# martende/findex

Measured on NVIDIA B200. Metric: fm_count_queries_per_s_len16_1GB_text, higher is better.
Workload: dtype u32

## Files before the change

findex_b200/csrc/fmx_device.cuh:

```cuda
#pragma once
#include <cstdint>
#include <cuda_runtime.h>

#include "../../include/fmgpu.h"

namespace fmx {

constexpr uint32_t kBitsPerBlock = 480;
constexpr int kCodeAbsent = 0xFF;

struct DevIndex {
    const uint4   *blocks;
    uint64_t       stride;
    const uint8_t *bwt;
    const uint32_t *C;
    const uint32_t *base;
    const uint8_t *code;
    const uint4   *mark;
    const uint32_t *samples;
    const uint4   *bm;
    uint32_t n, eof;
    int32_t  layout, levels;
    uint32_t z[8];
    int32_t  wmx_b, wmx_levels;
// ... 384 lines not shown
__device__ __forceinline__ bool dict_chain(const DevIndex &ix, const uint8_t *code, PatFn pat, int &i, uint32_t &sp, uint32_t &ep,
                                           uint32_t &touched, uint32_t &steps, int depth, bool top_known_missed = false) {
    const int Jc = ix.dict_Jc;
    const uint32_t bits = (uint32_t)ix.dict_bits;
    for (int t = (depth - ix.dict_D) / Jc + 1; t <= kDictMaxTiers && i >= 0 && depth < ix.dict_Dx; ++t) {
        const int j = (i + 1) < Jc ? (i + 1) : Jc;
        uint64_t syms = 0;
        bool ok = true;
        for (int k = 0; k < j; ++k) {
            const uint32_t c = pat(i - k), cd = code[c];
            ok = ok && (cd != (uint32_t)kCodeAbsent) && (c != 0);
            syms |= (uint64_t)cd << (bits * (uint32_t)k);
        }
        if (!ok) return true;
        uint32_t s, e;
        if (!top_known_missed && dict_probe<G, STATS>(ix, dict_chain_key(sp, j, t, syms), s, e, touched)) {
            sp = s; ep = e;
            i -= j;
            depth += j;
            if (STATS) steps += j;
            if (j < Jc) return true;
            continue;
        }
        if (!BISECT) return false;
        int lo = 0, hi = j - 1;
        uint32_t bs = 0, be = 0;
        const uint32_t psp = sp;
        while (lo < hi) {
            const int mid = (lo + hi + 1) >> 1;
            if (dict_probe<G, STATS>(ix, dict_chain_key(psp, mid, t, syms & ((1ull << (bits * (uint32_t)mid)) - 1ull)), s, e, touched)) { lo = mid; bs = s; be = e; }
            else hi = mid - 1;
        }
        if (lo > 0) { sp = bs; ep = be; i -= lo; if (STATS) steps += lo; }
        return true;
    }
    return true;
}

struct CtxQuery {
    unsigned long long qlo, qhi, mlo, mhi;
    uint32_t sh;
    bool zero, absent;
};
template <typename PatFn>
__device__ __forceinline__ CtxQuery ctx_query(const DevIndex &ix, const SharedTables &tb, PatFn pat, int j, int o) {
    CtxQuery q;
    const uint32_t bits = (uint32_t)ix.isat_bits;
    q.qlo = 0; q.qhi = 0;
    q.sh = (uint32_t)(ix.ctx_J - j) * bits;
    const uint32_t nb = (uint32_t)j * bits;
    q.mlo = nb >= 64 ? ~0ull : ((1ull << nb) - 1ull);
    q.mhi = nb <= 64 ? 0ull : ((1ull << (nb - 64)) - 1ull);
    q.zero = false; q.absent = false;
    if (ix.ctx_raw) {
        uint32_t w0, w1, w2;
        pat.bytes12(o, w0, w1, w2);
        q.qlo = ((unsigned long long)w1 << 32) | w0;
        q.qhi = w2;
        const unsigned long long l = q.qlo | ~q.mlo, h = (q.qhi & q.mhi) | ~q.mhi;
        q.zero = (((l - 0x0101010101010101ull) & ~l) | ((h - 0x0101010101010101ull) & ~h)) & 0x8080808080808080ull;
    } else {
        for (int k = 0; k < j; ++k) {
            const uint32_t pc = pat(o + k), cd = tb.code[pc];
            q.zero = q.zero || (pc == 0);
            q.absent = q.absent || (cd == (uint32_t)kCodeAbsent);
            const unsigned long long v = (unsigned long long)((cd + 1u) & ((1u << bits) - 1u));
            const uint32_t ob = (uint32_t)k * bits;
            if (ob < 64) { q.qlo |= v << ob; if (ob + bits > 64) q.qhi |= v >> (64 - ob); }
            else q.qhi |= v << (ob - 64);
        }
    }
    return q;
}
__device__ __forceinline__ bool ctx_match(const CtxQuery &q, const uint4 &b) {
    const unsigned long long elo = ((unsigned long long)b.z << 32) | b.y, ehi = b.w;
    unsigned long long lo, hi;
    if (q.sh == 0) { lo = elo; hi = ehi; }
    else if (q.sh < 64) { lo = (elo >> q.sh) | (ehi << (64 - q.sh)); hi = ehi >> q.sh; }
    else { lo = ehi >> (q.sh - 64); hi = 0; }
    return (((lo ^ q.qlo) & q.mlo) | ((hi ^ q.qhi) & q.mhi)) == 0ull;
}

constexpr uint32_t kKmerGroup = 8, kKmerWide = 0xFFu, kKmerInlineRows = 3;

template <int G, bool STATS, typename PatFn>
__device__ __forceinline__ void kmer_group(const DevIndex &ix, const SharedTables &tb, PatFn pat, bool fetch, uint32_t idx, int &i,
                                           uint32_t &sp, uint32_t &ep, uint32_t &touched, uint32_t &steps, uint32_t &pre_from,
                                           uint32_t &pre_best, uint32_t &pre_cnt) {
    const uint4 *blk = reinterpret_cast<const uint4 *>(ix.kmer) + (uint64_t)(idx / kKmerGroup) * 4;
    uint4 q0, q1, q2, q3;
    if constexpr (G == 1) {
        const uint32_t odd = threadIdx.x & 1u;
        const unsigned long long mine = reinterpret_cast<unsigned long long>(blk);
        const unsigned long long pe = __shfl_sync(0xFFFFFFFFu, mine, (threadIdx.x & 31u) & ~1u);
        const unsigned long long po = __shfl_sync(0xFFFFFFFFu, mine, (threadIdx.x & 31u) | 1u);
        const bool fe = __shfl_sync(0xFFFFFFFFu, fetch, (threadIdx.x & 31u) & ~1u), fo = __shfl_sync(0xFFFFFFFFu, fetch, (threadIdx.x & 31u) | 1u);
        uint4 x0 = make_uint4(0, 0, 0, 0), x1 = x0, y0 = x0, y1 = x0;
        if (fe) ldg256(reinterpret_cast<const uint4 *>(pe) + 2 * odd, x0, x1);
        if (fo) ldg256(reinterpret_cast<const uint4 *>(po) + 2 * odd, y0, y1);
        uint4 s0 = odd ? x0 : y0, s1 = odd ? x1 : y1;
        s0.x = __shfl_xor_sync(0xFFFFFFFFu, s0.x, 1); s0.y = __shfl_xor_sync(0xFFFFFFFFu, s0.y, 1);
        s0.z = __shfl_xor_sync(0xFFFFFFFFu, s0.z, 1); s0.w = __shfl_xor_sync(0xFFFFFFFFu, s0.w, 1);
        s1.x = __shfl_xor_sync(0xFFFFFFFFu, s1.x, 1); s1.y = __shfl_xor_sync(0xFFFFFFFFu, s1.y, 1);
        s1.z = __shfl_xor_sync(0xFFFFFFFFu, s1.z, 1); s1.w = __shfl_xor_sync(0xFFFFFFFFu, s1.w, 1);
        if (odd) { q0 = s0; q1 = s1; q2 = y0; q3 = y1; } else { q0 = x0; q1 = x1; q2 = s0; q3 = s1; }
    } else {
        if (!fetch) return;
        ldg256(blk, q0, q1);
        ldg256(blk + 2, q2, q3);
    }
    if (!fetch) return;
    const uint32_t e = idx % kKmerGroup, kind = q0.w >> 24, base = q0.x;
    uint32_t lo, hi;
    if (kind != kKmerWide) {
        const unsigned long long ends = ((unsigned long long)q0.z << 32) | q0.y;
        hi = base + (uint32_t)((ends >> (8 * e)) & 0xFFu);
        lo = base + (e ? (uint32_t)((ends >> (8 * e - 8)) & 0xFFu) : 0u);
    } else {
        auto end_of = [&](uint32_t k) {
            return k < 4 ? (k < 2 ? (k == 0 ? q1.x : q1.y) : (k == 2 ? q1.z : q1.w)) : (k < 6 ? (k == 4 ? q2.x : q2.y) : (k == 6 ? q2.z : q2.w));
        };
        hi = end_of(e);
        lo = (e ? end_of(e - 1) : base) + (((e < 4 ? q3.x : q3.y) >> (8 * (e & 3))) & 0xFFu);
    }
    if (lo < hi) { sp = lo; ep = hi; } else { sp = 0; ep = 0; }
    if (STATS) { touched += 1; steps += ix.kmer_k; }
    if (kind == kKmerWide || kind == 0 || ix.ctx == nullptr || sp >= ep || i < 0) return;
    const int rem = i + 1;
    const uint32_t rows = ep - sp;
    const int t = rem <= kCtxPlanMax ? (int)tb.plan[rem] : kCtxHops - 1;
    const uint32_t need = rem <= kCtxPlanMax ? (uint32_t)tb.plan[128 + rem] : (uint32_t)(rem / ix.ctx_J + 3);
    if (t != kCtxHops - 1 || rows > kCtxMaxRows || !(rows == 1u || rows * need <= (uint32_t)rem)) return;
    const int j = ix.ctx_J;
    const CtxQuery q = ctx_query(ix, tb, pat, j, rem - j);
    if (q.zero) return;
    uint32_t best = 0xFFFFFFFFu, cnt = 0;
#pragma unroll
    for (uint32_t k = 0; k < kKmerInlineRows; ++k) {
        const uint4 &pl = k == 0 ? q1 : k == 1 ? q2 : q3;
        if (k < kind && base + k >= sp && base + k < ep && !q.absent && ctx_match(q, pl)) { best = pl.x < best ? pl.x : best; ++cnt; }
    }
    if (ep <= base + kind) {
        if (cnt) { sp = best; ep = best + cnt; } else { sp = 0; ep = 0; }
        i -= j;
        if (STATS) steps += j;
    } else {
        const int lane = (G == 1) ? 0 : (threadIdx.x & (G - 1));
        pre_from = base + kind;
        pre_best = best;
        pre_cnt = lane == 0 ? cnt : 0u;
    }
}

constexpr int kSearchFresh = 0, kSearchTopMissed = 1, kSearchResume = 2, kSearchChainMissed = 3;
template <int G, int LAYOUT, bool STATS, typename PatFn>
__device__ __forceinline__ void search_pattern(const DevIndex &ix, const SharedTables &tb, PatFn pat, int len, bool active,
                                               uint32_t &sp, uint32_t &ep, uint32_t &touched, uint32_t &steps,
                                               int mode = kSearchFresh, uint32_t rsp = 0, uint32_t rep = 0, int rconsumed = 0) {
    const int lane = (G == 1) ? 0 : (threadIdx.x & (G - 1));
    const uint32_t gmask = group_mask<G>();
    sp = 0;
    ep = active ? ix.n : 0u;
    int i = len - 1;
    bool noshort = (ix.isat == nullptr);
    uint32_t pre_from = 0, pre_best = 0xFFFFFFFFu, pre_cnt = 0;
    bool kfetch = false;
    uint32_t kidx = 0;
    if (active && (mode == kSearchResume || mode == kSearchChainMissed)) {
        sp = rsp; ep = rep;
        i -= rconsumed;
        if (mode == kSearchChainMissed) dict_chain<G, STATS, true>(ix, tb.code, pat, i, sp, ep, touched, steps, rconsumed, true);
    } else if (active && i >= 0) {
        bool done = false;
        if (ix.dict != nullptr && len > ix.kmer_k) {
            const int K = ix.kmer_k;
            const uint32_t bits = (uint32_t)ix.dict_bits;
            int hi = len < ix.dict_D ? len : ix.dict_D;
            uint64_t full = 0;
            bool ok = true;
            for (int j = 0; j < hi; ++j) {
                const uint32_t c = pat(len - 1 - j), code = tb.code[c];
                ok = ok && (code != (uint32_t)kCodeAbsent) && (c != 0);
                full |= (uint64_t)code << (bits * (uint32_t)j);
            }
            if (ok) {
                int lo = K, d = hi;
                uint32_t bsp = 0, bep = 0;
                if (mode == kSearchTopMissed) { --hi; d = (lo + hi + 1) >> 1; }
                while (lo < hi) {
                    uint32_t s, e;
                    if (dict_probe<G, STATS>(ix, dict_key(full, d, bits), s, e, touched)) { lo = d; bsp = s; bep = e; }
                    else hi = d - 1;
                    d = (lo + hi + 1) >> 1;
                }
                if (lo > K) {
                    sp = bsp; ep = bep;
                    i -= lo;
                    done = true;
                    if (STATS) steps += lo;
                    if (lo == ix.dict_D && ix.dict_Dx > ix.dict_D) dict_chain<G, STATS, true>(ix, tb.code, pat, i, sp, ep, touched, steps, lo);
                }
            }
        }
        if (!done && ix.kmer != nullptr && len >= ix.kmer_k) {
            const int K = ix.kmer_k;
            uint32_t idx = 0;
            bool ok = true;
            for (int j = 0; j < K; ++j) {
                const uint32_t c = pat(ix.kmer_rows ? len - K + j : len - 1 - j), code = tb.code[c];
                ok = ok && (code != (uint32_t)kCodeAbsent) && (c != 0);
                idx = idx * ix.kmer_sigma + code;
            }
            if (ok) {
                i -= K;
                done = true;
                if (ix.kmer_rows) { kfetch = true; kidx = idx; }
                else {
                    const uint2 v = ldg64(ix.kmer + idx);
                    sp = v.x; ep = v.y;
                    if (STATS) { touched += 1; steps += K; }
                }
            }
        }
        if (!done) {
            const uint32_t c = pat(i);
            sp = tb.C[c];
            ep = tb.C[c + 1];
            --i;
            if (STATS) ++steps;
        }
    }
    if (ix.kmer != nullptr && ix.kmer_rows) kmer_group<G, STATS>(ix, tb, pat, kfetch, kidx, i, sp, ep, touched, steps, pre_from, pre_best, pre_cnt);
    bool noctx = (ix.ctx == nullptr && ix.ctx8 == nullptr);
    for (;;) {
        const bool go = (i >= 0) && (sp < ep);
        if (go) {
            bool stepped = false;
            const int rem = i + 1;
            if (!noctx && ix.ctx8 != nullptr && (ep - sp) <= kCtxMaxRows && rem >= ix.ctx8_J) {
                const int J = ix.ctx8_J, o = rem - J;
                uint32_t q = 0;
                bool zero = false, absent = false;
                for (int k = 0; k < J; ++k) {
                    const uint32_t pc = pat(o + k), cd = tb.code[pc];
                    zero = zero || (pc == 0);
                    absent = absent || (cd == (uint32_t)kCodeAbsent);
                    q |= (cd & 3u) << (2 * k);
                }
                if (zero) noctx = true;
                else {
                    uint32_t best = 0xFFFFFFFFu, cnt = 0;
                    if (!absent) {
                        for (uint32_t r = sp + (uint32_t)lane; r < ep; r += G) {
                            const uint2 e = ldg64(ix.ctx8 + r);
                            if (e.y == q && e.x != 0xFFFFFFFFu) { best = e.x < best ? e.x : best; ++cnt; }
                        }
                    }
                    if (STATS && lane == 0) { touched += absent ? 0u : ep - sp; steps += J; }
                    if (G >= 2) { best = min(best, __shfl_xor_sync(gmask, best, 1)); cnt += __shfl_xor_sync(gmask, cnt, 1); }
                    if (G >= 4) { best = min(best, __shfl_xor_sync(gmask, best, 2)); cnt += __shfl_xor_sync(gmask, cnt, 2); }
                    if (cnt) { sp = best; ep = best + cnt; } else { sp = 0; ep = 0; }
                    i -= J;
                    stepped = true;
                }
            }
            if (!stepped && !noctx && ix.ctx != nullptr && (ep - sp) <= kCtxMaxRows) {
                const uint32_t rows = ep - sp;
                const int t = rem <= kCtxPlanMax ? (int)tb.plan[rem] : kCtxHops - 1;
                const uint32_t need = rem <= kCtxPlanMax ? (uint32_t)tb.plan[128 + rem] : (uint32_t)(rem / ix.ctx_J + 3);
                if (rows == 1u || rows * need <= (uint32_t)rem) {
                    const int j = (int)tb.hops[t];
                    const CtxQuery q = ctx_query(ix, tb, pat, j, rem - j);
                    if (q.zero) noctx = true;
                    else {
                        const uint32_t from = sp > pre_from ? sp : pre_from;
                        uint32_t best = pre_best, cnt = pre_cnt;
                        if (!q.absent) {
                            for (uint32_t r = from + (uint32_t)lane; r < ep; r += G) {
                                uint4 a, b;
                                ldg256(ix.ctx + (uint64_t)r * 2, a, b);
                                if (ctx_match(q, b)) {
                                    const uint32_t row = t == 0 ? a.x : t == 1 ? a.y : t == 2 ? a.z : t == 3 ? a.w : b.x;
                                    best = row < best ? row : best;
                                    ++cnt;
                                }
                            }
                        }
                        pre_from = 0; pre_best = 0xFFFFFFFFu; pre_cnt = 0;
                        if (STATS && lane == 0) { touched += q.absent ? 0u : ep - from; steps += j; }
                        if (G >= 2) { best = min(best, __shfl_xor_sync(gmask, best, 1)); cnt += __shfl_xor_sync(gmask, cnt, 1); }
                        if (G >= 4) { best = min(best, __shfl_xor_sync(gmask, best, 2)); cnt += __shfl_xor_sync(gmask, cnt, 2); }
                        if (cnt) { sp = best; ep = best + cnt; } else { sp = 0; ep = 0; }
                        i -= j;
                        stepped = true;
                    }
                }
            }
            if (!stepped && !noshort && (ep - sp) == 1u && i >= 2 && i < ix.isat_syms) {
                const uint32_t q = ldg32(ix.sa + sp);
                const bool fits = q >= (uint32_t)rem;
                const uint32_t b0 = fits ? q - (uint32_t)rem : 0u;
                const uint4 e = ldg128(ix.isat + b0);
                const uint32_t bits = (uint32_t)ix.isat_bits, fmask = (1u << bits) - 1u;
                bool eq = fits, zero = false;
                for (int k = lane; k < rem; k += G) {
                    const uint32_t pc = pat(k);
                    const uint32_t o = (uint32_t)k * bits, w = o >> 5;
                    const uint32_t lo = w == 0 ? e.y : w == 1 ? e.z : e.w, hi = w == 0 ? e.z : w == 1 ? e.w : 0u;
                    const uint32_t sym = __funnelshift_r(lo, hi, o & 31u) & fmask;
                    zero = zero || (pc == 0);
                    eq = eq && (sym == (uint32_t)tb.code[pc] + 1u);
                }
                if (G > 1) { eq = __all_sync(gmask, eq); zero = __any_sync(gmask, zero); }
                if (zero) noshort = true;
                else {
                    if (eq) { sp = e.x; ep = e.x + 1; } else { sp = 0; ep = 0; }
                    i = -1;
                    stepped = true;
                    if (STATS) { touched += 2; steps += rem; }
                }
            }
            if (!stepped) {
                backward_step<G, LAYOUT, STATS>(ix, tb, pat(i), sp, ep, touched);
                --i;
                if (STATS) ++steps;
            }
        }
        if (__all_sync(0xFFFFFFFFu, !go)) break;
    }
}

template <int G, int LAYOUT>
__device__ __forceinline__ uint32_t lf_value(const DevIndex &ix, const SharedTables &t, uint32_t c, uint32_t pos) {
    const uint32_t code = t.code[c];
    if (c == 0) return pos > ix.eof ? 1u : 0u;
    if (code == kCodeAbsent) return t.C[c];
    if (LAYOUT == FMX_LAYOUT_PLANES) {
        return t.base[c] + rank_one<G>(ix.blocks + (uint64_t)code * ix.stride * 4, pos, nullptr);
    } else if (LAYOUT == FMX_LAYOUT_WMX) {
        uint32_t p = pos;
        const int b = ix.wmx_b, L = ix.wmx_levels;
        for (int l = 0; l < L; ++l) {
            const uint32_t d = (code >> (b * (L - 1 - l))) & ((1u << b) - 1u);
            p = ix.zx[l][d] + rank_one_x<G>(ix.blocks + (uint64_t)l * ix.wmx_stride * 8, b, d, p);
        }
        if (code == 0) p -= (pos > ix.eof);
        return t.base[c] + p;
    } else {
        uint32_t p = pos;
        const int L = ix.levels;
        for (int l = 0; l < L; ++l) {
            uint32_t r = rank_one<G>(ix.blocks + (uint64_t)l * ix.stride * 4, p, nullptr);
            if ((code >> (L - 1 - l)) & 1u) p = ix.z[l] + r; else p -= r;
        }
        if (code == 0) p -= (pos > ix.eof);
        return t.base[c] + p;
    }
}

}
```

findex_b200/csrc/fmx_kernels.cu:

```cuda
#include "fmx_kernels.cuh"

#include <algorithm>

namespace fmx {

template <int G, int LAYOUT, bool STATS, typename OutT, int MINB = (LAYOUT == FMX_LAYOUT_WMX ? 5 : (G == 1) ? 6 : 8)>
__global__ void __launch_bounds__(kThreads, MINB)
count_fixed_kernel(const __grid_constant__ DevIndex ix, const uint8_t *__restrict__ pat, int len, long long m,
                   OutT *__restrict__ sp_out, OutT *__restrict__ ep_out, unsigned long long *stats, const __grid_constant__ PeerSinks sinks) {
    __shared__ SharedTables tb;
    extern __shared__ __align__(16) uint8_t spat[];
    constexpr int QPB = kThreads / G;
    load_tables(tb, ix);

    const long long q0 = (long long)blockIdx.x * QPB;
    const int nq = (int)((m - q0) < (long long)QPB ? (m - q0) : (long long)QPB);
    {
        const uint8_t *src = pat + q0 * len;
        const int nbytes = nq * len;
        if ((reinterpret_cast<uintptr_t>(src) & 15) == 0) {
            const int nvec = nbytes >> 4;
            for (int i = threadIdx.x; i < nvec; i += kThreads)
                reinterpret_cast<uint4 *>(spat)[i] = ldg128(reinterpret_cast<const uint4 *>(src) + i);
            for (int i = (nvec << 4) + threadIdx.x; i < nbytes; i += kThreads) spat[i] = src[i];
        } else {
            for (int i = threadIdx.x; i < nbytes; i += kThreads) spat[i] = src[i];
        }
    }
    __syncthreads();

    const int g = threadIdx.x / G;
    const bool active = g < nq;
    uint32_t sp, ep, touched = 0, steps = 0;
    search_pattern<G, LAYOUT, STATS>(ix, tb, SmemPattern{spat + g * len, len, (len & 3) == 0}, len, active, sp, ep, touched, steps);
    const bool hit = sp < ep;
    const uint32_t cnt = hit ? ep - sp : 0u;
    if (active && (threadIdx.x % G) == 0) {
        sp_out[q0 + g] = hit ? (OutT)sp : (OutT)0;
        ep_out[q0 + g] = hit ? (OutT)ep : (OutT)0;
        if (sinks.n == 1) sinks.p[0][sinks.offset + q0 + g] = cnt;
    }
    if (sinks.n > 1) {
        __shared__ __align__(16) uint32_t scnt[kThreads];
        if ((threadIdx.x % G) == 0) scnt[g] = active ? cnt : 0u;
        __syncthreads();
        const long long base = sinks.offset + q0;
        if (nq == QPB && (base & 3) == 0) {
            constexpr int V = QPB / 4;
            for (int w = threadIdx.x; w < sinks.n * V; w += kThreads) {
                const int j = w / V, k = w - j * V;
                reinterpret_cast<uint4 *>(sinks.p[j] + base)[k] = reinterpret_cast<const uint4 *>(scnt)[k];
            }
        } else {
            for (int w = threadIdx.x; w < sinks.n * nq; w += kThreads) {
                const int j = w / nq, k = w - j * nq;
                sinks.p[j][base + k] = scnt[k];
            }
        }
    }
    if (STATS) {
        if ((threadIdx.x % G) != 0) { touched = 0; steps = 0; }
        for (int o = 16; o; o >>= 1) {
            touched += __shfl_xor_sync(0xFFFFFFFFu, touched, o);
            steps += __shfl_xor_sync(0xFFFFFFFFu, steps, o);
        }
        if ((threadIdx.x & 31) == 0) { atomicAdd(&stats[0], (unsigned long long)touched); atomicAdd(&stats[1], (unsigned long long)steps); }
    }
}

template <int G, int LAYOUT, typename OutT>
__global__ void __launch_bounds__(kThreads)
count_fixed_gmem_kernel(const __grid_constant__ DevIndex ix, const uint8_t *__restrict__ pat, int len, long long m, OutT *__restrict__ sp_out,
                        OutT *__restrict__ ep_out, const __grid_constant__ PeerSinks sinks) {
    __shared__ SharedTables tb;
    load_tables(tb, ix);
    __syncthreads();
    constexpr int QPB = kThreads / G;
    const long long q = (long long)blockIdx.x * QPB + threadIdx.x / G;
    const bool active = q < m;
    uint32_t sp, ep, touched = 0, steps = 0;
    search_pattern<G, LAYOUT, false>(ix, tb, GlobalPattern{pat + (active ? q : 0) * len, len}, len, active, sp, ep, touched, steps);
    if (active && (threadIdx.x % G) == 0) {
        const bool hit = sp < ep;
        sp_out[q] = hit ? (OutT)sp : (OutT)0;
        ep_out[q] = hit ? (OutT)ep : (OutT)0;
        for (int j = 0; j < sinks.n; ++j) sinks.p[j][sinks.offset + q] = hit ? ep - sp : 0u;
    }
}

constexpr uint32_t kListModeShift = 30, kListIdMask = (1u << kListModeShift) - 1u;

template <typename OutT>
__global__ void __launch_bounds__(kThreads)
count_dict_first_kernel(const __grid_constant__ DevIndex ix, const uint8_t *__restrict__ pat, int len, long long m, OutT *__restrict__ sp_out,
                        OutT *__restrict__ ep_out, uint2 *__restrict__ list, unsigned long long *__restrict__ list_count,
                        const __grid_constant__ PeerSinks sinks) {
    __shared__ uint8_t scode[256];
    extern __shared__ __align__(16) uint8_t spat[];
    for (int i = threadIdx.x; i < 256; i += kThreads) scode[i] = ix.code[i];
    const int d0 = len < ix.dict_D ? len : ix.dict_D;
    const long long q0 = (long long)blockIdx.x * kThreads;
    const int nq = (int)((m - q0) < (long long)kThreads ? (m - q0) : (long long)kThreads);
    {
        const uint8_t *src = pat + q0 * len;
        const int nbytes = nq * len;
        if ((reinterpret_cast<uintptr_t>(src) & 15) == 0) {
            const int nvec = nbytes >> 4;
            for (int i = threadIdx.x; i < nvec; i += kThreads)
                reinterpret_cast<uint4 *>(spat)[i] = ldg128(reinterpret_cast<const uint4 *>(src) + i);
            for (int i = (nvec << 4) + threadIdx.x; i < nbytes; i += kThreads) spat[i] = src[i];
        } else {
            for (int i = threadIdx.x; i < nbytes; i += kThreads) spat[i] = src[i];
        }
    }
    __syncthreads();
    const bool active = (int)threadIdx.x < nq;
    const long long q = q0 + threadIdx.x;
    uint32_t entry = 0xFFFFFFFFu, consumed = 0;
    if (active) {
        const uint8_t *p = spat + (size_t)threadIdx.x * len;
        const uint32_t bits = (uint32_t)ix.dict_bits;
        uint64_t full = 0;
        bool ok = true;
        for (int j = 0; j < d0; ++j) {
            const uint32_t c = p[len - 1 - j], code = scode[c];
            ok = ok && (code != (uint32_t)kCodeAbsent) && (c != 0);
            full |= (uint64_t)code << (bits * (uint32_t)j);
        }
        entry = (uint32_t)threadIdx.x | ((uint32_t)kSearchFresh << kListModeShift);
        if (ok) {
            uint32_t s = 0, e = 0, touched = 0;
            if (dict_probe<1, false>(ix, dict_key(full, d0, bits), s, e, touched)) {
                int i = len - 1 - d0;
                bool chain_open = true;
                if (i >= 0 && ix.dict_Dx > ix.dict_D) {
                    uint32_t steps = 0;
                    chain_open = dict_chain<1, false, false>(ix, scode, SmemPattern{p, len, false}, i, s, e, touched, steps, d0);
                }
                consumed = (uint32_t)(len - 1 - i);
                sp_out[q] = (OutT)s;
                ep_out[q] = (OutT)e;
                if (i < 0) {
                    entry = 0xFFFFFFFFu;
                    for (int j = 0; j < sinks.n; ++j) sinks.p[j][sinks.offset + q] = e - s;
                } else entry = (uint32_t)threadIdx.x | ((uint32_t)(chain_open ? kSearchResume : kSearchChainMissed) << kListModeShift);
            } else entry = (uint32_t)threadIdx.x | ((uint32_t)kSearchTopMissed << kListModeShift);
        }
    }
    __shared__ uint32_t wcount[kThreads / 32];
    __shared__ unsigned long long cta_base;
    const uint32_t need = __ballot_sync(0xFFFFFFFFu, entry != 0xFFFFFFFFu);
    const int lane = threadIdx.x & 31, warp = threadIdx.x >> 5;
    if (lane == 0) wcount[warp] = (uint32_t)__popc(need);
    __syncthreads();
    if (threadIdx.x == 0) {
        uint32_t total = 0;
        for (int w = 0; w < kThreads / 32; ++w) { const uint32_t c = wcount[w]; wcount[w] = total; total += c; }
        cta_base = total ? atomicAdd(list_count, (unsigned long long)total) : 0ull;
    }
    __syncthreads();
    if (entry != 0xFFFFFFFFu) {
        const uint32_t mode = entry >> kListModeShift;
        list[cta_base + wcount[warp] + __popc(need & ((1u << lane) - 1u))] = make_uint2((uint32_t)(q0 + (entry & kListIdMask)) | (mode << kListModeShift), consumed);
    }
}

template <int G, int LAYOUT, typename OutT>
__global__ void __launch_bounds__(kThreads)
count_list_kernel(const __grid_constant__ DevIndex ix, const uint8_t *__restrict__ pat, int len, OutT *__restrict__ sp_out, OutT *__restrict__ ep_out,
                  const uint2 *__restrict__ list, const unsigned long long *__restrict__ list_count, const __grid_constant__ PeerSinks sinks) {
    __shared__ SharedTables tb;
    extern __shared__ __align__(16) uint8_t spat[];
    constexpr int QPB = kThreads / G;
    const unsigned long long count = *list_count;
    if ((unsigned long long)blockIdx.x * QPB >= count) return;
    load_tables(tb, ix);
    const int g = threadIdx.x / G, lane = threadIdx.x % G;
    const int stride = (len + 3) & ~3;
    {
        const unsigned long long t = (unsigned long long)blockIdx.x * QPB + g;
        const bool active = t < count;
        const uint2 le = active ? list[t] : make_uint2(0u, 0u);
        const uint32_t entry = le.x;
        const long long q = (long long)(entry & kListIdMask);
        const int mode = (int)(entry >> kListModeShift);
        __syncthreads();
        if (active) {
            const uint8_t *src = pat + q * len;
            uint8_t *dst = spat + (size_t)g * stride;
            if ((len & 3) == 0 && (reinterpret_cast<uintptr_t>(src) & 3) == 0)
                for (int w = lane; w < (len >> 2); w += G) reinterpret_cast<uint32_t *>(dst)[w] = __ldg(reinterpret_cast<const uint32_t *>(src) + w);
            else
                for (int b = lane; b < len; b += G) dst[b] = __ldg(src + b);
        }
        __syncthreads();
        uint32_t rsp = 0, rep = 0;
        if (active && (mode == kSearchResume || mode == kSearchChainMissed)) { rsp = (uint32_t)sp_out[q]; rep = (uint32_t)ep_out[q]; }
        uint32_t sp, ep, touched = 0, steps = 0;
        search_pattern<G, LAYOUT, false>(ix, tb, SmemPattern{spat + (size_t)g * stride, len, true}, len, active, sp, ep, touched, steps, mode, rsp, rep, (int)le.y);
        if (active && (threadIdx.x % G) == 0) {
            const bool hit = sp < ep;
            sp_out[q] = hit ? (OutT)sp : (OutT)0;
            ep_out[q] = hit ? (OutT)ep : (OutT)0;
            for (int j = 0; j < sinks.n; ++j) sinks.p[j][sinks.offset + q] = hit ? ep - sp : 0u;
        }
    }
}

template <int G, int LAYOUT>
__global__ void __launch_bounds__(kThreads)
count_var_kernel(const __grid_constant__ DevIndex ix, const uint8_t *__restrict__ pat, const long long *__restrict__ off,
                 long long m, long long *__restrict__ sp_out, long long *__restrict__ ep_out) {
    __shared__ SharedTables tb;
    load_tables(tb, ix);
    __syncthreads();
    constexpr int QPB = kThreads / G;
    const long long q = (long long)blockIdx.x * QPB + threadIdx.x / G;
    const bool active = q < m;
    long long lo = 0, hi = 0;
// ... 177 lines not shown
        if (++k > ix.n) { FMX_EMIT(0xFFFFFFFFu); return; }
    }
#undef FMX_EMIT
}

template <typename OutT>
__global__ void key_positions_kernel(const unsigned long long *__restrict__ key, long long n, OutT *__restrict__ out) {
    const long long i = (long long)blockIdx.x * blockDim.x + threadIdx.x;
    if (i < n) out[i] = (OutT)(key[i] & 0xFFFFFFFFull);
}
cudaError_t launch_key_positions(const uint64_t *d_key, int64_t n, uint32_t *d_out32, int64_t *d_out64, cudaStream_t st) {
    if (n <= 0) return cudaSuccess;
    const unsigned grid = (unsigned)((n + 255) / 256);
    if (d_out32) key_positions_kernel<uint32_t><<<grid, 256, 0, st>>>((const unsigned long long *)d_key, n, d_out32);
    else key_positions_kernel<long long><<<grid, 256, 0, st>>>((const unsigned long long *)d_key, n, (long long *)d_out64);
    return cudaGetLastError();
}

__global__ void unpack2_kernel(const uint8_t *__restrict__ codes, int len, long long m, uint32_t alpha4, uint8_t *__restrict__ out) {
    const int pb = (len + 3) >> 2;
    const long long t = (long long)blockIdx.x * blockDim.x + threadIdx.x;
    if (t >= m * pb) return;
    const long long q = t / pb;
    const int b = (int)(t - q * pb);
    const uint32_t c = codes[t];
    uint8_t *dst = out + q * len + 4 * b;
#pragma unroll
    for (int j = 0; j < 4; ++j)
        if (4 * b + j < len) dst[j] = (uint8_t)(alpha4 >> (8 * ((c >> (2 * j)) & 3u)));
}
cudaError_t launch_unpack2(const uint8_t *d_codes, int len, int64_t m, uint32_t alpha4, uint8_t *d_out, cudaStream_t st) {
    const int64_t total = m * ((len + 3) / 4);
    if (total > 0) unpack2_kernel<<<(unsigned)((total + 255) / 256), 256, 0, st>>>(d_codes, len, m, alpha4, d_out);
    return cudaGetLastError();
}

__global__ void interval_len_kernel(const uint32_t *__restrict__ sp, const uint32_t *__restrict__ ep, long long m, long long *__restrict__ out) {
    const long long q = (long long)blockIdx.x * blockDim.x + threadIdx.x;
    if (q > m) return;
    out[q] = (q < m && ep[q] > sp[q]) ? (long long)(ep[q] - sp[q]) : 0ll;
}
cudaError_t launch_interval_len(const uint32_t *d_sp, const uint32_t *d_ep, int64_t m, int64_t *d_out, cudaStream_t st) {
    interval_len_kernel<<<(unsigned)((m + 1 + 255) / 256), 256, 0, st>>>(d_sp, d_ep, m, (long long *)d_out);
    return cudaGetLastError();
}

__global__ void __launch_bounds__(256)
scatter_words_kernel(const uint32_t *__restrict__ src, long long count, const __grid_constant__ PeerSinks sinks, const long long *__restrict__ d_dst_off,
                     long long dst_scale) {
    const long long dst0 = sinks.offset + (d_dst_off ? *d_dst_off * dst_scale : 0ll);
    const long long stride = (long long)gridDim.x * blockDim.x, tid = (long long)blockIdx.x * blockDim.x + threadIdx.x;
    if (((reinterpret_cast<uintptr_t>(src) | (uintptr_t)(dst0 * 4)) & 15) == 0) {
        const long long nv = count >> 2;
        for (long long i = tid; i < nv; i += stride) {
            const uint4 v = reinterpret_cast<const uint4 *>(src)[i];
            for (int j = 0; j < sinks.n; ++j) reinterpret_cast<uint4 *>(sinks.p[j] + dst0)[i] = v;
        }
        for (long long i = (nv << 2) + tid; i < count; i += stride) { const uint32_t v = src[i]; for (int j = 0; j < sinks.n; ++j) sinks.p[j][dst0 + i] = v; }
    } else {
        for (long long i = tid; i < count; i += stride) { const uint32_t v = src[i]; for (int j = 0; j < sinks.n; ++j) sinks.p[j][dst0 + i] = v; }
    }
}
cudaError_t launch_scatter_words(const uint32_t *d_src, int64_t count, const PeerSinks &sinks, const int64_t *d_dst_off, int64_t dst_scale, cudaStream_t st) {
    if (count <= 0 || sinks.n <= 0) return cudaSuccess;
    const unsigned grid = (unsigned)std::min<int64_t>((count / 4 + 255) / 256 + 1, 148 * 8);
    scatter_words_kernel<<<grid, 256, 0, st>>>(d_src, count, sinks, (const long long *)d_dst_off, dst_scale);
    return cudaGetLastError();
}

template <int LANES, int VEC>
__global__ void __launch_bounds__(kThreads)
gather_kernel(const uint4 *__restrict__ base, unsigned long long n_units, long long gathers, int chain, uint32_t seed,
              unsigned long long *sink) {
    const long long gid = ((long long)blockIdx.x * kThreads + threadIdx.x) / LANES;
    const int lane = threadIdx.x % LANES;
    if (gid >= gathers) return;
    unsigned long long x = (unsigned long long)gid * 0x9E3779B97F4A7C15ull + seed;
    uint32_t acc = 0;
    for (int s = 0; s < chain; ++s) {
        x ^= x >> 33; x *= 0xFF51AFD7ED558CCDull; x ^= x >> 33; x *= 0xC4CEB9FE1A85EC53ull; x ^= x >> 33;
        const unsigned long long unit = __umul64hi(x, n_units);
        const uint4 *p = base + unit * (LANES * VEC) + lane * VEC;
        uint32_t v = 0;
#pragma unroll
        for (int i = 0; i < VEC; ++i) { const uint4 q = ldg128(p + i); v ^= q.x ^ q.y ^ q.z ^ q.w; }
        if (LANES > 1) {
            const uint32_t mask = ((LANES == 32) ? 0xFFFFFFFFu : ((1u << LANES) - 1u)) << ((threadIdx.x & 31) & ~(LANES - 1));
            for (int o = 1; o < LANES; o <<= 1) v ^= __shfl_xor_sync(mask, v, o);
        }
        acc ^= v;
        x += v;
    }
    if (acc == 0x12345678u && lane == 0) atomicAdd(sink, 1ull);
}

#define FMX_DISPATCH(cfg, CALL)                                                                      \
    do {                                                                                             \
        if ((cfg).layout == FMX_LAYOUT_PLANES) {                                                     \
            if ((cfg).lanes == 1) { CALL(1, FMX_LAYOUT_PLANES); }                                    \
            else if ((cfg).lanes == 2) { CALL(2, FMX_LAYOUT_PLANES); }                               \
            else { CALL(4, FMX_LAYOUT_PLANES); }                                                     \
        } else if ((cfg).layout == FMX_LAYOUT_WMX) {                                                 \
            if ((cfg).lanes == 1) { CALL(1, FMX_LAYOUT_WMX); }                                       \
            else if ((cfg).lanes == 2) { CALL(2, FMX_LAYOUT_WMX); }                                  \
            else { CALL(4, FMX_LAYOUT_WMX); }                                                        \
        } else {                                                                                     \
            if ((cfg).lanes == 1) { CALL(1, FMX_LAYOUT_WM); }                                        \
            else if ((cfg).lanes == 2) { CALL(2, FMX_LAYOUT_WM); }                                   \
            else { CALL(4, FMX_LAYOUT_WM); }                                                         \
        }                                                                                            \
    } while (0)

static inline unsigned grid_for(int64_t items, int lanes) {
    const int64_t per = kThreads / lanes;
    return (unsigned)((items + per - 1) / per);
}

cudaError_t launch_count_fixed(const DevIndex &ix, LaunchCfg cfg, const uint8_t *d_pat, int len, int64_t m, void *d_sp,
                               void *d_ep, bool out64, unsigned long long *d_stats, cudaStream_t st, const PeerSinks *sinks_or_null) {
    if (m <= 0) return cudaSuccess;
    if (cfg.count_lanes) cfg.lanes = cfg.count_lanes;
    PeerSinks sinks{};
    if (sinks_or_null) sinks = *sinks_or_null;
    const size_t smem = (size_t)(kThreads / cfg.lanes) * (size_t)(len > 0 ? len : 1) + 16;
    const bool too_long = smem > 160 * 1024;
    if (ix.dict != nullptr && len > ix.kmer_k && len <= ix.dict_Dx && !d_stats && m < (1ll << kListModeShift) && (size_t)kThreads * (size_t)len <= 160 * 1024) {
        unsigned long long *cnt = nullptr;
        cudaError_t e = cudaMallocAsync(&cnt, 16 + (size_t)m * 8, st);
        if (e != cudaSuccess) return e;
        uint2 *list = reinterpret_cast<uint2 *>(cnt + 2);
        cudaMemsetAsync(cnt, 0, 8, st);
        const size_t smem1 = (size_t)kThreads * (size_t)len;
        const unsigned grid1 = grid_for(m, 1);
        if (out64) {
            auto k = count_dict_first_kernel<long long>;
            cudaFuncSetAttribute(k, cudaFuncAttributeMaxDynamicSharedMemorySize, (int)smem1);
            k<<<grid1, kThreads, smem1, st>>>(ix, d_pat, len, m, (long long *)d_sp, (long long *)d_ep, list, cnt, sinks);
        } else {
            auto k = count_dict_first_kernel<uint32_t>;
            cudaFuncSetAttribute(k, cudaFuncAttributeMaxDynamicSharedMemorySize, (int)smem1);
            k<<<grid1, kThreads, smem1, st>>>(ix, d_pat, len, m, (uint32_t *)d_sp, (uint32_t *)d_ep, list, cnt, sinks);
        }
        const unsigned grid2 = grid_for(m, cfg.lanes);
#define CALL2(G, LAY)                                                                                                  \
        {                                                                                                              \
            const size_t smem2 = (size_t)(kThreads / G) * (size_t)((len + 3) & ~3) + 16;                               \
            if (out64) count_list_kernel<G, LAY, long long><<<grid2, kThreads, smem2, st>>>(ix, d_pat, len, (long long *)d_sp, (long long *)d_ep, list, cnt, sinks); \
            else count_list_kernel<G, LAY, uint32_t><<<grid2, kThreads, smem2, st>>>(ix, d_pat, len, (uint32_t *)d_sp, (uint32_t *)d_ep, list, cnt, sinks); \
        }
        FMX_DISPATCH(cfg, CALL2);
#undef CALL2
        cudaFreeAsync(cnt, st);
        return cudaGetLastError();
    }
#define CALL(G, LAY)                                                                                                  \
    {                                                                                                                 \
        if (too_long && !d_stats) {                                                                                   \
            if (out64) count_fixed_gmem_kernel<G, LAY, long long><<<grid_for(m, G), kThreads, 0, st>>>(ix, d_pat, len, m, (long long *)d_sp, (long long *)d_ep, sinks); \
            else count_fixed_gmem_kernel<G, LAY, uint32_t><<<grid_for(m, G), kThreads, 0, st>>>(ix, d_pat, len, m, (uint32_t *)d_sp, (uint32_t *)d_ep, sinks); \
        } else if (too_long) {                                                                                        \
            return cudaErrorInvalidValue;                                                                             \
        } else if (d_stats) {                                                                                                \
            auto k = count_fixed_kernel<G, LAY, true, uint32_t>;                                                      \
            cudaFuncSetAttribute(k, cudaFuncAttributeMaxDynamicSharedMemorySize, (int)smem);                          \
            k<<<grid_for(m, G), kThreads, smem, st>>>(ix, d_pat, len, m, (uint32_t *)d_sp, (uint32_t *)d_ep, d_stats, sinks); \
        } else if (out64) {                                                                                           \
            auto k = count_fixed_kernel<G, LAY, false, long long>;                                                    \
            cudaFuncSetAttribute(k, cudaFuncAttributeMaxDynamicSharedMemorySize, (int)smem);                          \
            k<<<grid_for(m, G), kThreads, smem, st>>>(ix, d_pat, len, m, (long long *)d_sp, (long long *)d_ep, nullptr, sinks); \
        } else if (cfg.min_blocks >= 4 && cfg.min_blocks <= 8) {                      \
            auto k = cfg.min_blocks == 4 ? count_fixed_kernel<G, LAY, false, uint32_t, 4> : cfg.min_blocks == 5 ? count_fixed_kernel<G, LAY, false, uint32_t, 5> : \
                     cfg.min_blocks == 6 ? count_fixed_kernel<G, LAY, false, uint32_t, 6> : cfg.min_blocks == 7 ? count_fixed_kernel<G, LAY, false, uint32_t, 7> : \
                     count_fixed_kernel<G, LAY, false, uint32_t, 8>;                                                  \
            cudaFuncSetAttribute(k, cudaFuncAttributeMaxDynamicSharedMemorySize, (int)smem);                          \
            k<<<grid_for(m, G), kThreads, smem, st>>>(ix, d_pat, len, m, (uint32_t *)d_sp, (uint32_t *)d_ep, nullptr, sinks); \
        } else {                                                                                                      \
            auto k = count_fixed_kernel<G, LAY, false, uint32_t>;                                                     \
            cudaFuncSetAttribute(k, cudaFuncAttributeMaxDynamicSharedMemorySize, (int)smem);                          \
            k<<<grid_for(m, G), kThreads, smem, st>>>(ix, d_pat, len, m, (uint32_t *)d_sp, (uint32_t *)d_ep, nullptr, sinks); \
        }                                                                                                             \
    }
    FMX_DISPATCH(cfg, CALL);
#undef CALL
    return cudaGetLastError();
}

cudaError_t launch_count_var(const DevIndex &ix, LaunchCfg cfg, const uint8_t *d_pat, const int64_t *d_off, int64_t m,
                             int64_t *d_sp, int64_t *d_ep, cudaStream_t st) {
    if (m <= 0) return cudaSuccess;
    if (cfg.count_lanes) cfg.lanes = cfg.count_lanes;
#define CALL(G, LAY) count_var_kernel<G, LAY><<<grid_for(m, G), kThreads, 0, st>>>(ix, d_pat, (const long long *)d_off, m, (long long *)d_sp, (long long *)d_ep)
    FMX_DISPATCH(cfg, CALL);
#undef CALL
    return cudaGetLastError();
}

cudaError_t launch_occ(const DevIndex &ix, LaunchCfg cfg, const uint8_t *d_c, const int64_t *d_key, int64_t m, int64_t *d_out,
                       cudaStream_t st) {
    if (m <= 0) return cudaSuccess;
#define CALL(G, LAY) occ_kernel<G, LAY><<<grid_for(m, G), kThreads, 0, st>>>(ix, d_c, (const long long *)d_key, m, (long long *)d_out)
    FMX_DISPATCH(cfg, CALL);
#undef CALL
    return cudaGetLastError();
}

cudaError_t launch_prev_range(const DevIndex &ix, LaunchCfg cfg, const int64_t *d_sp, const int64_t *d_ep, const uint8_t *d_c,
                              int64_t m, int64_t *d_sp1, int64_t *d_ep1, cudaStream_t st) {
    if (m <= 0) return cudaSuccess;
#define CALL(G, LAY) prev_range_kernel<G, LAY><<<grid_for(m, G), kThreads, 0, st>>>(ix, (const long long *)d_sp, (const long long *)d_ep, d_c, m, (long long *)d_sp1, (long long *)d_ep1)
    FMX_DISPATCH(cfg, CALL);
#undef CALL
    return cudaGetLastError();
}

cudaError_t launch_interval_prev_range(const DevIndex &ix, LaunchCfg cfg, int64_t sp, int64_t ep, int cstart, int cend,
                                       int64_t *d_sp1, int64_t *d_ep1, cudaStream_t st) {
    const int64_t m = cend - cstart + 1;
    if (m <= 0) return cudaSuccess;
#define CALL(G, LAY) interval_prev_range_kernel<G, LAY><<<grid_for(m, G), kThreads, 0, st>>>(ix, (uint32_t)sp, (uint32_t)ep, cstart, cend, (long long *)d_sp1, (long long *)d_ep1)
    FMX_DISPATCH(cfg, CALL);
#undef CALL
    return cudaGetLastError();
}

cudaError_t launch_lf(const DevIndex &ix, LaunchCfg cfg, const int64_t *d_row, int64_t m, int64_t *d_out, cudaStream_t st) {
    if (m <= 0) return cudaSuccess;
#define CALL(G, LAY) lf_kernel<G, LAY><<<grid_for(m, G), kThreads, 0, st>>>(ix, (const long long *)d_row, m, (long long *)d_out)
    FMX_DISPATCH(cfg, CALL);
#undef CALL
    return cudaGetLastError();
}

cudaError_t launch_prev_substr(const DevIndex &ix, LaunchCfg cfg, const int64_t *d_row, int64_t m, int len, uint8_t *d_out,
                               cudaStream_t st) {
    if (m <= 0 || len <= 0) return cudaSuccess;
#define CALL(G, LAY) prev_substr_kernel<G, LAY><<<grid_for(m, G), kThreads, 0, st>>>(ix, (const long long *)d_row, m, len, d_out)
    FMX_DISPATCH(cfg, CALL);
#undef CALL
    return cudaGetLastError();
}

cudaError_t launch_fl(const DevIndex &ix, LaunchCfg cfg, const int64_t *d_row, int64_t m, int64_t *d_out, cudaStream_t st) {
    if (m <= 0) return cudaSuccess;
#define CALL(G, LAY) fl_kernel<G, LAY><<<grid_for(m, G), kThreads, 0, st>>>(ix, (const long long *)d_row, m, (long long *)d_out)
    FMX_DISPATCH(cfg, CALL);
#undef CALL
    return cudaGetLastError();
}

cudaError_t launch_next_substr(const DevIndex &ix, LaunchCfg cfg, const int64_t *d_row, int64_t m, int len, uint8_t *d_out,
                               int *d_out_len, cudaStream_t st) {
    if (m <= 0) return cudaSuccess;
#define CALL(G, LAY) next_substr_kernel<G, LAY><<<grid_for(m, G), kThreads, 0, st>>>(ix, (const long long *)d_row, m, len, d_out, d_out_len)
    FMX_DISPATCH(cfg, CALL);
#undef CALL
    return cudaGetLastError();
}

cudaError_t launch_locate(const DevIndex &ix, LaunchCfg cfg, const uint32_t *d_sp, const int64_t *d_off, int64_t q0, int64_t q1,
                          int64_t t0, int64_t count, uint32_t *d_pos, uint64_t *d_key, unsigned long long *d_steps, cudaStream_t st) {
    if (count <= 0) return cudaSuccess;
#define CALL(G, LAY) locate_kernel<G, LAY><<<grid_for(count, G), kThreads, 0, st>>>(ix, d_sp, (const long long *)d_off, q0, q1, t0, count, d_pos, (unsigned long long *)d_key, d_steps)
    FMX_DISPATCH(cfg, CALL);
#undef CALL
    return cudaGetLastError();
}

cudaError_t launch_gather_bench(const uint4 *base, uint64_t n_blocks64, int bytes, int lanes, int64_t gathers, int chain,
                                uint32_t seed, unsigned long long *d_sink, cudaStream_t st) {
    const int per_lane = bytes / lanes;
    if (per_lane < 16 || per_lane % 16 || (per_lane / 16) > 8 || lanes < 1 || lanes > 32 || (lanes & (lanes - 1))) return cudaErrorInvalidValue;
    const int vec = per_lane / 16;
    const unsigned long long units = n_blocks64 * 64ull / (unsigned long long)bytes;
    const unsigned grid = (unsigned)((gathers * lanes + kThreads - 1) / kThreads);
#define GK(L, V) gather_kernel<L, V><<<grid, kThreads, 0, st>>>(base, units, gathers, chain, seed, d_sink)
    if (vec == 1) { switch (lanes) { case 1: GK(1, 1); break; case 2: GK(2, 1); break; case 4: GK(4, 1); break; case 8: GK(8, 1); break; case 16: GK(16, 1); break; default: GK(32, 1); } }
    else if (vec == 2) { switch (lanes) { case 1: GK(1, 2); break; case 2: GK(2, 2); break; case 4: GK(4, 2); break; case 8: GK(8, 2); break; default: return cudaErrorInvalidValue; } }
    else if (vec == 4) { switch (lanes) { case 1: GK(1, 4); break; case 2: GK(2, 4); break; case 4: GK(4, 4); break; default: return cudaErrorInvalidValue; } }
    else if (vec == 8) { switch (lanes) { case 1: GK(1, 8); break; case 2: GK(2, 8); break; default: return cudaErrorInvalidValue; } }
    else return cudaErrorInvalidValue;
#undef GK
    return cudaGetLastError();
}

}
```

Measured before the change: 27.40 billion.

## Add persistent warp kernel that compacts unfinished queries into a queue

Adds a persistent count kernel in which each warp stages tiles of 32 patterns into shared memory with cp.async double buffering. It resolves each pattern's k-mer prefix, writes finished queries immediately, and compacts the remaining ones into a per-warp queue. The backward search runs only when 32 queued queries are ready, so all lanes stay busy. The goal is to cut warp divergence from queries that finish early and to overlap pattern loads with compute, at the cost of extra shared memory and queue bookkeeping.

Measured after the change: 28.36 billion, median of 6. 1.03x the previous value.

```diff
diff --git a/findex_b200/csrc/fmx_device.cuh b/findex_b200/csrc/fmx_device.cuh
--- a/findex_b200/csrc/fmx_device.cuh
+++ b/findex_b200/csrc/fmx_device.cuh
@@ -560,85 +560,25 @@
     }
 }
 
-constexpr int kSearchFresh = 0, kSearchTopMissed = 1, kSearchResume = 2, kSearchChainMissed = 3;
+template <typename PatFn>
+__device__ __forceinline__ bool kmer_entry(const DevIndex &ix, const SharedTables &tb, PatFn pat, int len, uint32_t &idx) {
+    const int K = ix.kmer_k;
+    idx = 0;
+    bool ok = true;
+    for (int j = 0; j < K; ++j) {
+        const uint32_t c = pat(ix.kmer_rows ? len - K + j : len - 1 - j), code = tb.code[c];
+        ok = ok && (code != (uint32_t)kCodeAbsent) && (c != 0);
+        idx = idx * ix.kmer_sigma + code;
+    }
+    return ok;
+}
+
 template <int G, int LAYOUT, bool STATS, typename PatFn>
-__device__ __forceinline__ void search_pattern(const DevIndex &ix, const SharedTables &tb, PatFn pat, int len, bool active,
-                                               uint32_t &sp, uint32_t &ep, uint32_t &touched, uint32_t &steps,
-                                               int mode = kSearchFresh, uint32_t rsp = 0, uint32_t rep = 0, int rconsumed = 0) {
+__device__ __forceinline__ void search_rest(const DevIndex &ix, const SharedTables &tb, PatFn pat, int i, uint32_t &sp, uint32_t &ep,
+                                            uint32_t pre_from, uint32_t pre_best, uint32_t pre_cnt, uint32_t &touched, uint32_t &steps) {
     const int lane = (G == 1) ? 0 : (threadIdx.x & (G - 1));
     const uint32_t gmask = group_mask<G>();
-    sp = 0;
-    ep = active ? ix.n : 0u;
-    int i = len - 1;
     bool noshort = (ix.isat == nullptr);
-    uint32_t pre_from = 0, pre_best = 0xFFFFFFFFu, pre_cnt = 0;
-    bool kfetch = false;
-    uint32_t kidx = 0;
-    if (active && (mode == kSearchResume || mode == kSearchChainMissed)) {
-        sp = rsp; ep = rep;
-        i -= rconsumed;
-        if (mode == kSearchChainMissed) dict_chain<G, STATS, true>(ix, tb.code, pat, i, sp, ep, touched, steps, rconsumed, true);
-    } else if (active && i >= 0) {
-        bool done = false;
-        if (ix.dict != nullptr && len > ix.kmer_k) {
-            const int K = ix.kmer_k;
-            const uint32_t bits = (uint32_t)ix.dict_bits;
-            int hi = len < ix.dict_D ? len : ix.dict_D;
-            uint64_t full = 0;
-            bool ok = true;
-            for (int j = 0; j < hi; ++j) {
-                const uint32_t c = pat(len - 1 - j), code = tb.code[c];
-                ok = ok && (code != (uint32_t)kCodeAbsent) && (c != 0);
-                full |= (uint64_t)code << (bits * (uint32_t)j);
-            }
-            if (ok) {
-                int lo = K, d = hi;
-                uint32_t bsp = 0, bep = 0;
-                if (mode == kSearchTopMissed) { --hi; d = (lo + hi + 1) >> 1; }
-                while (lo < hi) {
-                    uint32_t s, e;
-                    if (dict_probe<G, STATS>(ix, dict_key(full, d, bits), s, e, touched)) { lo = d; bsp = s; bep = e; }
-                    else hi = d - 1;
-                    d = (lo + hi + 1) >> 1;
-                }
-                if (lo > K) {
-                    sp = bsp; ep = bep;
-                    i -= lo;
-                    done = true;
-                    if (STATS) steps += lo;
-                    if (lo == ix.dict_D && ix.dict_Dx > ix.dict_D) dict_chain<G, STATS, true>(ix, tb.code, pat, i, sp, ep, touched, steps, lo);
-                }
-            }
-        }
-        if (!done && ix.kmer != nullptr && len >= ix.kmer_k) {
-            const int K = ix.kmer_k;
-            uint32_t idx = 0;
-            bool ok = true;
-            for (int j = 0; j < K; ++j) {
-                const uint32_t c = pat(ix.kmer_rows ? len - K + j : len - 1 - j), code = tb.code[c];
-                ok = ok && (code != (uint32_t)kCodeAbsent) && (c != 0);
-                idx = idx * ix.kmer_sigma + code;
-            }
-            if (ok) {
-                i -= K;
-                done = true;
-                if (ix.kmer_rows) { kfetch = true; kidx = idx; }
-                else {
-                    const uint2 v = ldg64(ix.kmer + idx);
-                    sp = v.x; ep = v.y;
-                    if (STATS) { touched += 1; steps += K; }
-                }
-            }
-        }
-        if (!done) {
-            const uint32_t c = pat(i);
-            sp = tb.C[c];
-            ep = tb.C[c + 1];
-            --i;
-            if (STATS) ++steps;
-        }
-    }
-    if (ix.kmer != nullptr && ix.kmer_rows) kmer_group<G, STATS>(ix, tb, pat, kfetch, kidx, i, sp, ep, touched, steps, pre_from, pre_best, pre_cnt);
     bool noctx = (ix.ctx == nullptr && ix.ctx8 == nullptr);
     for (;;) {
         const bool go = (i >= 0) && (sp < ep);
@@ -738,6 +678,79 @@
     }
 }
 
+constexpr int kSearchFresh = 0, kSearchTopMissed = 1, kSearchResume = 2, kSearchChainMissed = 3;
+template <int G, int LAYOUT, bool STATS, typename PatFn>
+__device__ __forceinline__ void search_pattern(const DevIndex &ix, const SharedTables &tb, PatFn pat, int len, bool active,
+                                               uint32_t &sp, uint32_t &ep, uint32_t &touched, uint32_t &steps,
+                                               int mode = kSearchFresh, uint32_t rsp = 0, uint32_t rep = 0, int rconsumed = 0) {
+    sp = 0;
+    ep = active ? ix.n : 0u;
+    int i = len - 1;
+    uint32_t pre_from = 0, pre_best = 0xFFFFFFFFu, pre_cnt = 0;
+    bool kfetch = false;
+    uint32_t kidx = 0;
+    if (active && (mode == kSearchResume || mode == kSearchChainMissed)) {
+        sp = rsp; ep = rep;
+        i -= rconsumed;
+        if (mode == kSearchChainMissed) dict_chain<G, STATS, true>(ix, tb.code, pat, i, sp, ep, touched, steps, rconsumed, true);
+    } else if (active && i >= 0) {
+        bool done = false;
+        if (ix.dict != nullptr && len > ix.kmer_k) {
+            const int K = ix.kmer_k;
+            const uint32_t bits = (uint32_t)ix.dict_bits;
+            int hi = len < ix.dict_D ? len : ix.dict_D;
+            uint64_t full = 0;
+            bool ok = true;
+            for (int j = 0; j < hi; ++j) {
+                const uint32_t c = pat(len - 1 - j), code = tb.code[c];
+                ok = ok && (code != (uint32_t)kCodeAbsent) && (c != 0);
+                full |= (uint64_t)code << (bits * (uint32_t)j);
+            }
+            if (ok) {
+                int lo = K, d = hi;
+                uint32_t bsp = 0, bep = 0;
+                if (mode == kSearchTopMissed) { --hi; d = (lo + hi + 1) >> 1; }
+                while (lo < hi) {
+                    uint32_t s, e;
+                    if (dict_probe<G, STATS>(ix, dict_key(full, d, bits), s, e, touched)) { lo = d; bsp = s; bep = e; }
+                    else hi = d - 1;
+                    d = (lo + hi + 1) >> 1;
+                }
+                if (lo > K) {
+                    sp = bsp; ep = bep;
+                    i -= lo;
+                    done = true;
+                    if (STATS) steps += lo;
+                    if (lo == ix.dict_D && ix.dict_Dx > ix.dict_D) dict_chain<G, STATS, true>(ix, tb.code, pat, i, sp, ep, touched, steps, lo);
+                }
+            }
+        }
+        if (!done && ix.kmer != nullptr && len >= ix.kmer_k) {
+            const int K = ix.kmer_k;
+            uint32_t idx;
+            if (kmer_entry(ix, tb, pat, len, idx)) {
+                i -= K;
+                done = true;
+                if (ix.kmer_rows) { kfetch = true; kidx = idx; }
+                else {
+                    const uint2 v = ldg64(ix.kmer + idx);
+                    sp = v.x; ep = v.y;
+                    if (STATS) { touched += 1; steps += K; }
+                }
+            }
+        }
+        if (!done) {
+            const uint32_t c = pat(i);
+            sp = tb.C[c];
+            ep = tb.C[c + 1];
+            --i;
+            if (STATS) ++steps;
+        }
+    }
+    if (ix.kmer != nullptr && ix.kmer_rows) kmer_group<G, STATS>(ix, tb, pat, kfetch, kidx, i, sp, ep, touched, steps, pre_from, pre_best, pre_cnt);
+    search_rest<G, LAYOUT, STATS>(ix, tb, pat, i, sp, ep, pre_from, pre_best, pre_cnt, touched, steps);
+}
+
 template <int G, int LAYOUT>
 __device__ __forceinline__ uint32_t lf_value(const DevIndex &ix, const SharedTables &t, uint32_t c, uint32_t pos) {
     const uint32_t code = t.code[c];
diff --git a/findex_b200/csrc/fmx_kernels.cu b/findex_b200/csrc/fmx_kernels.cu
--- a/findex_b200/csrc/fmx_kernels.cu
+++ b/findex_b200/csrc/fmx_kernels.cu
@@ -65,6 +65,136 @@
             steps += __shfl_xor_sync(0xFFFFFFFFu, steps, o);
         }
         if ((threadIdx.x & 31) == 0) { atomicAdd(&stats[0], (unsigned long long)touched); atomicAdd(&stats[1], (unsigned long long)steps); }
+    }
+}
+
+constexpr int kGroupTile = 32;
+constexpr int kGroupQueue = 2 * kGroupTile;
+constexpr int kGroupMinBlocks = 4;
+
+struct GroupSmem {
+    int stage, qstride, qpat, per_warp;
+    __host__ __device__ explicit GroupSmem(int len) {
+        stage = ((kGroupTile * len + 15) & ~15) + 16;
+        qstride = (len + 3) & ~3;
+        qpat = ((kGroupQueue * qstride + 15) & ~15) + 16;
+        per_warp = 2 * stage + qpat + 6 * kGroupQueue * 4;
+    }
+};
+enum { kQeQuery, kQeSp, kQeEp, kQeRest, kQeFrom, kQeBest };
+
+__device__ __forceinline__ void cp_async16(void *dst, const void *src) {
+    asm volatile("cp.async.cg.shared.global [%0], [%1], 16;" :: "r"((uint32_t)__cvta_generic_to_shared(dst)), "l"(src) : "memory");
+}
+__device__ __forceinline__ void cp_async_commit() { asm volatile("cp.async.commit_group;" ::: "memory"); }
+__device__ __forceinline__ void cp_async_wait_prev() { asm volatile("cp.async.wait_group 1;" ::: "memory"); }
+__device__ __forceinline__ void cp_async_wait_all() { asm volatile("cp.async.wait_all;" ::: "memory"); }
+
+__device__ __forceinline__ void stage_tile(uint8_t *dst, const uint8_t *pat, uint32_t t, int len, long long m, int lane) {
+    const long long q0 = (long long)t * kGroupTile;
+    const int nbytes = (int)(((m - q0) < kGroupTile ? (m - q0) : kGroupTile) * len);
+    const uint8_t *src = pat + q0 * len;
+    int done = 0;
+    if ((reinterpret_cast<uintptr_t>(src) & 15) == 0) {
+        const int nvec = nbytes >> 4;
+        for (int v = lane; v < nvec; v += 32) cp_async16(dst + 16 * v, src + 16 * v);
+        done = nvec << 4;
+    }
+    for (int b = done + lane; b < nbytes; b += 32) dst[b] = src[b];
+}
+
+template <typename OutT>
+__device__ __forceinline__ void store_count(OutT *sp_out, OutT *ep_out, const PeerSinks &sinks, long long q, uint32_t sp, uint32_t ep) {
+    const bool hit = sp < ep;
+    sp_out[q] = hit ? (OutT)sp : (OutT)0;
+    ep_out[q] = hit ? (OutT)ep : (OutT)0;
+    if (sinks.n == 1) sinks.p[0][sinks.offset + q] = hit ? ep - sp : 0u;
+}
+
+template <int LAYOUT, bool STATS, typename OutT>
+__device__ __forceinline__ void drain_queue(const DevIndex &ix, const SharedTables &tb, const uint8_t *qpat, const uint32_t *qe, int qstride,
+                                            int len, int first, int n, OutT *sp_out, OutT *ep_out, const PeerSinks &sinks, uint32_t &touched,
+                                            uint32_t &steps) {
+    const int lane = threadIdx.x & 31, e = first + lane;
+    const bool active = lane < n;
+    uint32_t sp = 0, ep = 0, from = 0, best = 0xFFFFFFFFu, cnt = 0, q = 0;
+    int i = -1;
+    if (active) {
+        q = qe[kQeQuery * kGroupQueue + e]; sp = qe[kQeSp * kGroupQueue + e]; ep = qe[kQeEp * kGroupQueue + e];
+        const uint32_t r = qe[kQeRest * kGroupQueue + e];
+        i = (int)(r & 0xFFFFu); cnt = r >> 16;
+        from = qe[kQeFrom * kGroupQueue + e]; best = qe[kQeBest * kGroupQueue + e];
+    }
+    search_rest<1, LAYOUT, STATS>(ix, tb, SmemPattern{qpat + (size_t)e * qstride, len, true}, i, sp, ep, from, best, cnt, touched, steps);
+    if (active) store_count(sp_out, ep_out, sinks, (long long)q, sp, ep);
+}
+
+template <int LAYOUT, bool STATS, typename OutT>
+__global__ void __launch_bounds__(kThreads, kGroupMinBlocks)
+count_group_kernel(const __grid_constant__ DevIndex ix, const uint8_t *__restrict__ pat, int len, long long m,
+                   OutT *__restrict__ sp_out, OutT *__restrict__ ep_out, unsigned long long *stats, const __grid_constant__ PeerSinks sinks) {
+    __shared__ SharedTables tb;
+    extern __shared__ __align__(16) uint8_t gsm[];
+    load_tables(tb, ix);
+    __syncthreads();
+    constexpr int kWarps = kThreads / 32;
+    const GroupSmem L(len);
+    const int lane = threadIdx.x & 31;
+    uint8_t *const wsm = gsm + (size_t)(threadIdx.x >> 5) * L.per_warp;
+    uint8_t *const qpat = wsm + 2 * L.stage;
+    uint32_t *const qe = reinterpret_cast<uint32_t *>(qpat + L.qpat);
+    const uint32_t lt = (1u << lane) - 1u;
+    const uint32_t tiles = (uint32_t)((m + kGroupTile - 1) / kGroupTile);
+    uint32_t t = blockIdx.x * kWarps + (threadIdx.x >> 5);
+    uint32_t touched = 0, steps = 0;
+    int qn = 0;
+    if (t < tiles) stage_tile(wsm, pat, t, len, m, lane);
+    cp_async_commit();
+    for (int b = 0; t < tiles; t += gridDim.x * kWarps, b ^= 1) {
+        const uint32_t next = t + gridDim.x * kWarps;
+        if (next < tiles) stage_tile(wsm + (b ^ 1) * L.stage, pat, next, len, m, lane);
+        cp_async_commit();
+        cp_async_wait_prev();
+        __syncwarp();
+        const uint32_t q = t * kGroupTile + lane;
+        const bool active = q < m;
+        const uint8_t *const p = wsm + b * L.stage + lane * len;
+        const SmemPattern P{p, len, (len & 3) == 0};
+        uint32_t sp = 0, ep = active ? ix.n : 0u, from = 0, best = 0xFFFFFFFFu, cnt = 0, kidx = 0;
+        int i = len - 1;
+        bool kfetch = false;
+        if (active && i >= 0) {
+            if (len >= ix.kmer_k && kmer_entry(ix, tb, P, len, kidx)) { i -= ix.kmer_k; kfetch = true; }
+            else { const uint32_t c = P(i); sp = tb.C[c]; ep = tb.C[c + 1]; --i; if (STATS) ++steps; }
+        }
+        kmer_group<1, STATS>(ix, tb, P, kfetch, kidx, i, sp, ep, touched, steps, from, best, cnt);
+        const bool more = active && i >= 0 && sp < ep;
+        if (active && !more) store_count(sp_out, ep_out, sinks, q, sp, ep);
+        const uint32_t want = __ballot_sync(0xFFFFFFFFu, more);
+        if (more) {
+            const int e = qn + __popc(want & lt);
+            qe[kQeQuery * kGroupQueue + e] = q; qe[kQeSp * kGroupQueue + e] = sp; qe[kQeEp * kGroupQueue + e] = ep;
+            qe[kQeRest * kGroupQueue + e] = (uint32_t)i | (cnt << 16); qe[kQeFrom * kGroupQueue + e] = from; qe[kQeBest * kGroupQueue + e] = best;
+            uint8_t *dst = qpat + (size_t)e * L.qstride;
+            if ((len & 3) == 0) for (int w = 0; w < (len >> 2); ++w) reinterpret_cast<uint32_t *>(dst)[w] = reinterpret_cast<const uint32_t *>(p)[w];
+            else for (int k = 0; k < len; ++k) dst[k] = p[k];
+        }
+        qn += __popc(want);
+        __syncwarp();
+        if (qn >= kGroupTile) {
+            qn -= kGroupTile;
+            drain_queue<LAYOUT, STATS>(ix, tb, qpat, qe, L.qstride, len, qn, kGroupTile, sp_out, ep_out, sinks, touched, steps);
+        }
+        __syncwarp();
+    }
+    cp_async_wait_all();
+    drain_queue<LAYOUT, STATS>(ix, tb, qpat, qe, L.qstride, len, 0, qn, sp_out, ep_out, sinks, touched, steps);
+    if (STATS) {
+        for (int o = 16; o; o >>= 1) {
+            touched += __shfl_xor_sync(0xFFFFFFFFu, touched, o);
+            steps += __shfl_xor_sync(0xFFFFFFFFu, steps, o);
+        }
+        if (lane == 0) { atomicAdd(&stats[0], (unsigned long long)touched); atomicAdd(&stats[1], (unsigned long long)steps); }
     }
 }
 
@@ -548,6 +678,34 @@
 #undef CALL2
         cudaFreeAsync(cnt, st);
         return cudaGetLastError();
+    }
+    if (ix.kmer != nullptr && ix.kmer_rows > 0 && ix.dict == nullptr && cfg.lanes == 1 && sinks.n <= 1 && m <= (int64_t)UINT32_MAX &&
+        (cfg.layout == FMX_LAYOUT_PLANES || cfg.layout == FMX_LAYOUT_WM)) {
+        const size_t gsmem = (size_t)(kThreads / 32) * (size_t)GroupSmem(len).per_warp;
+        void (*k)(const DevIndex, const uint8_t *, int, long long, uint32_t *, uint32_t *, unsigned long long *, const PeerSinks) = nullptr;
+        void (*k64)(const DevIndex, const uint8_t *, int, long long, long long *, long long *, unsigned long long *, const PeerSinks) = nullptr;
+        const bool planes = cfg.layout == FMX_LAYOUT_PLANES;
+        if (out64) k64 = planes ? count_group_kernel<FMX_LAYOUT_PLANES, false, long long> : count_group_kernel<FMX_LAYOUT_WM, false, long long>;
+        else if (d_stats) k = planes ? count_group_kernel<FMX_LAYOUT_PLANES, true, uint32_t> : count_group_kernel<FMX_LAYOUT_WM, true, uint32_t>;
+        else k = planes ? count_group_kernel<FMX_LAYOUT_PLANES, false, uint32_t> : count_group_kernel<FMX_LAYOUT_WM, false, uint32_t>;
+        const void *kf = out64 ? (const void *)k64 : (const void *)k;
+        int dev = 0, sms = 0, smem_max = 0, per_sm = 0;
+        cudaError_t e = cudaGetDevice(&dev);
+        if (e == cudaSuccess) e = cudaDeviceGetAttribute(&sms, cudaDevAttrMultiProcessorCount, dev);
+        if (e == cudaSuccess) e = cudaDeviceGetAttribute(&smem_max, cudaDevAttrMaxSharedMemoryPerBlockOptin, dev);
+        if (e != cudaSuccess) return e;
+        if (gsmem <= (size_t)smem_max) {
+            e = cudaFuncSetAttribute(kf, cudaFuncAttributeMaxDynamicSharedMemorySize, (int)gsmem);
+            if (e == cudaSuccess) e = cudaOccupancyMaxActiveBlocksPerMultiprocessor(&per_sm, kf, kThreads, gsmem);
+            if (e != cudaSuccess) return e;
+        }
+        if (per_sm >= kGroupMinBlocks) {
+            const int64_t warps = (m + kGroupTile - 1) / kGroupTile;
+            const unsigned grid = (unsigned)std::min<int64_t>((int64_t)per_sm * sms, (warps + kThreads / 32 - 1) / (kThreads / 32));
+            if (out64) k64<<<grid, kThreads, gsmem, st>>>(ix, d_pat, len, m, (long long *)d_sp, (long long *)d_ep, nullptr, sinks);
+            else k<<<grid, kThreads, gsmem, st>>>(ix, d_pat, len, m, (uint32_t *)d_sp, (uint32_t *)d_ep, d_stats, sinks);
+            return cudaGetLastError();
+        }
     }
 #define CALL(G, LAY)                                                                                                  \
     {                                                                                                                 \
```
